# hangelwen/miR-PREFeR

Measured on AMD Instinct MI355X. Metric: precursor windows folded+filtered/sec (L=300), higher is better.
Workload: dtype int16/int32 (energies in 0.01 kcal/mol)

## Files before the change

mir-prefer_amd/csrc/fold_lds_common.h:

```cpp
#pragma once
#include <hip/hip_runtime.h>
#include <type_traits>
#include <tuple>
#include <cstdio>
#include "fold_epilogue.h"
#include "fold185_device.h"

namespace mirp {

#define LNT 1024
#define LNT2 512
#define LCAP 352
#define LDMAX 300
#define LSPAN 300
#define I16_INF 0x7fff
#define FIN_LIMIT 28000
#define FML_BIAS 31500
#define FML_MAX 1267
#define LSEG 384
#define KEY_BIAS 40000
#define KEY_NONE 0xffffffffu
#define KEY_INF (65535u << 10)
#define OTH_BIAS 2048

// ... 2 lines not shown
    short bulge[32];
    short internal_loop[32];
    short mismatchI[200], mismatchH[200], mismatchM[200], mismatch1nI[200], mismatch23I[200];
    unsigned char XB[176];
    unsigned char X1[176];
    short dangle5[40], dangle3[40];
    unsigned char rt2[28];
    short ML_closing, ML_intern, TerminalAU, ninio, MAX_NINIO, pad[3];
};
__host__ __device__ constexpr int xt_pslot(int s) { return s == 3 ? 3 : s == 4 ? 4 : 0; }
__host__ __device__ constexpr int xt_qslot(int s) { return s == 1 ? 1 : s == 3 ? 2 : s == 4 ? 1 : 0; }
__host__ __device__ constexpr int xt_pcode(int sp, int sp_m1) { return xt_pslot(sp) * 25 + sp_m1; }
__host__ __device__ constexpr int xt_qcode(int sq, int sq_p1) { return xt_qslot(sq) * 25 + sq_p1 * 5; }
static_assert(xt_pslot(1) + xt_qslot(4) == 1 && xt_pslot(2) + xt_qslot(3) == 2 && xt_pslot(3) + xt_qslot(2) == 3 && xt_pslot(3) + xt_qslot(4) == 4 &&
              xt_pslot(4) + xt_qslot(1) == 5 && xt_pslot(4) + xt_qslot(3) == 6, "inner-pair table slots");
template <class TAB>
__device__ inline void xt_fill(TAB& T, const FoldParams* __restrict__ P, int tid, int nt) {
    for (int x = tid; x < 175; x += nt) {
        const int slot = x / 25, a = (x % 25) / 5, b = x % 5;
        const int sp = slot == 1 ? 1 : slot == 2 ? 2 : (slot == 3 || slot == 4) ? 3 : 4, sq = slot == 1 ? 4 : slot == 2 ? 3 : slot == 3 ? 2 : slot == 4 ? 4 : slot == 5 ? 1 : 3;
        const int t2 = slot ? rtype_of(pair_type(sp, sq)) : 0;
        int xb = 0, x1 = 0;
        if (t2) {
            const int mi = P->mismatchI[t2][a][b];
            xb = (t2 > 2 ? P->TerminalAU : 0) - mi;
            x1 = P->mismatch1nI[t2][a][b] - mi;
        }
        T.XB[x] = (unsigned char)(xb + P->xb_bias); T.X1[x] = (unsigned char)(x1 + P->x1_bias);
    }
}
#define CSTR MIRP_RING_CSTR
#define MIRP_CK(d) ((d) % 3)
#define CRING_ROWS 33

struct LTab {
    static constexpr bool kTiled = true;
    const short* fml;
    const int* off;
    const short* carch;
    const unsigned short* tb;
    __device__ __forceinline__ int at(int d, int i) const { return off[(i - 1) >> 3] + ((i - 1) & 7) + 8 * (d - 4); }
    __device__ __forceinline__ int TB(int d, int i) const { return tb[at(d, i)]; }
    __device__ __forceinline__ int C(int d, int i) const { int v = carch[at(d, i)]; return v == I16_INF ? INF : v; }
    __device__ __forceinline__ int TBat(int o) const { return tb[o]; }
    __device__ __forceinline__ int Cat(int o) const { int v = carch[o]; return v == I16_INF ? INF : v; }
    __device__ __forceinline__ int Mat(int o) const { const int v = (unsigned short)fml[o]; return v == 65535 ? INF : v - FML_BIAS; }
    __device__ __forceinline__ int M(int d, int i) const {
        if (d < 4) return INF;
        const int v = (unsigned short)fml[at(d, i)];
        return v == 65535 ? INF : v - FML_BIAS;
    }
};

__device__ __forceinline__ int lds_mlstem(const LdsTables& T, const FoldParams* __restrict__ P, int type, int a, int b) {
    int e = T.ML_intern + (type > 2 ? T.TerminalAU : 0);
    if (a >= 0 && b >= 0) e += T.mismatchM[type * 25 + a * 5 + b];
    else if (a >= 0) e += P->dangle5[type][a];
    else if (b >= 0) e += P->dangle3[type][b];
    return e;
}

__device__ __forceinline__ int lds_intloop(const LdsTables& T, const FoldParams* __restrict__ P, int n1, int n2, int type, int type2,
                                           int si1, int sj1, int sp1, int sq1) {
    int nl = n1 > n2 ? n1 : n2, ns = n1 > n2 ? n2 : n1;
    if (nl == 0) return T.stack[type * 8 + type2];
    if (ns == 0) {
// ... 11 lines not shown
    }
    if (ns == 2) {
        if (nl == 2) return P->int22[type][type2][si1][sp1][sq1][sj1];
        if (nl == 3) return T.internal_loop[5] + T.ninio + T.mismatch23I[type * 25 + si1 * 5 + sj1] + T.mismatch23I[type2 * 25 + sq1 * 5 + sp1];
    }
    int x = (nl - ns) * T.ninio;
    return T.internal_loop[nl + ns] + (x < T.MAX_NINIO ? x : T.MAX_NINIO) + T.mismatchI[type * 25 + si1 * 5 + sj1] +
           T.mismatchI[type2 * 25 + sq1 * 5 + sp1];
}

__host__ __device__ constexpr int tri_off(int d, int n) { return 1 + (d - 4) * n - (d * (d - 1) / 2 - 6) + (((d - 4) + (n & 1)) >> 1); }
__host__ __device__ constexpr int tri_len(int d, int n) { return n - d > 0 ? (n - d) + ((n - d) & 1) : 0; }
__host__ __device__ constexpr int tri_len_any(int d, int n) { return (n - d) + ((n - d) & 1); }
__device__ inline void fill_tri_off(int* off, int n) {
    int o = 1;
    for (int d = 4; d <= LDMAX + 1; d++) { off[d] = o; o += tri_len(d, n); }
}

#define ARCH_RB ((LCAP + 7) / 8)
__host__ __device__ constexpr int arch_nd(int b, int n, int dcap) {
    int m = n - 1 - 8 * b;
    if (m > dcap) m = dcap;
    m -= 3;
    return m > 0 ? (m + 7) & ~7 : 0;
}
__host__ __device__ inline int arch_rowblk_off(int b, int n, int dcap) {
    int o = 0;
    for (int x = 0; x < b; x++) o += 8 * arch_nd(x, n, dcap);
    return o;
}

struct LdsLayout {
    unsigned fml, aux, S, seq, pax, qb2, list, tabs, misc, total, fml_bytes, code4, spec;
};
#define CODE_STR 384
static_assert(CODE_STR % 16 == 0 && (LCAP - 2) - 5 + MAXLOOP + 3 < CODE_STR, "pair-code reads of the first diagonals stay inside their copy");
__host__ __device__ constexpr unsigned lds_al(unsigned x) { return (x + 15u) & ~15u; }
#define FML_REGION_BYTES (lds_al((tri_off(LDMAX + 1, LCAP - 2) + 2) * 2))
#define POOL_MIN_CAP 1024
#define FRING_STR (LCAP + 2)
#ifndef MIRP_FILL_TWO_BYTES
#define MIRP_FILL_TWO_BYTES 71680
#endif
#ifndef MIRP_OVERLAP_EPI_WGS
#define MIRP_OVERLAP_EPI_WGS 1
#endif
#define MIRP_OVERLAP_EPI_LDS (16u * 1280u)
#define LDS_GRANULES(b) (((b) + 1279u) / 1280u)
#define LDS_TWO_BYTES ((unsigned)(MIRP_FILL_TWO_BYTES))
static_assert(2u * LDS_GRANULES(LDS_TWO_BYTES) + MIRP_OVERLAP_EPI_WGS * LDS_GRANULES(MIRP_OVERLAP_EPI_LDS) <= 128u, "two fill workgroups and the epilogue workgroups beside them share one CU's 160 KB");
template <int MODEL, bool SPARSE = false, bool TWO = false>
__host__ __device__ constexpr LdsLayout lds_layout() {
    static_assert(!TWO || (SPARSE && MODEL == 0), "two windows per CU: candidate-pool pass of the default model only");
    LdsLayout L{};
    unsigned o = 0;
    if (!SPARSE) { L.fml = o; L.fml_bytes = FML_REGION_BYTES; o += L.fml_bytes; }
    L.aux = o; o += lds_al(CRING_ROWS * CSTR * 2 + (MODEL ? 5 : 3) * LCAP * 2 + (SPARSE ? 6 : 5) * LCAP * 4);
    L.S = o; o += lds_al(LCAP + 8);
    L.seq = o; o += lds_al(LCAP + 8);
    if (SPARSE) {
        L.code4 = o; L.qb2 = o; L.pax = o + 4 * CODE_STR; o += 8 * CODE_STR;
    } else {
        L.pax = o; o += CODE_STR;
        L.qb2 = o; o += CODE_STR;
    }
    L.list = o; o += lds_al(3 * LSEG * 4);
    L.tabs = o; o += lds_al((unsigned)sizeof(LdsTables));
    L.misc = o; o += lds_al((48 + ARCH_RB + ((SPARSE && MODEL) ? 48 : 0)) * 4);
    if (TWO) { L.spec = o; o += lds_al(3 * CSTR * 2); }
    if (SPARSE) { L.fml = o; L.fml_bytes = (TWO ? LDS_TWO_BYTES : 160u * 1024u) - o; o += L.fml_bytes; }
    L.total = o;
    return L;
}
static_assert(lds_layout<0>().total <= 160 * 1024 && lds_layout<1>().total <= 160 * 1024, "fill kernel LDS budget");
static_assert(lds_layout<0, true, true>().total <= LDS_TWO_BYTES, "two workgroups of the candidate-pool pass must fit one CU's 160 KB");
static_assert((lds_layout<0, true, true>().fml_bytes - lds_al(2 * FRING_STR * 2)) / 6 >= 2 * POOL_MIN_CAP, "two-per-CU layout: room for the candidate pool behind the fML ring");

typedef const volatile __attribute__((address_space(3))) unsigned short* lds_vu16;
typedef const volatile __attribute__((address_space(3))) unsigned char* lds_vu8;
typedef const volatile __attribute__((address_space(3))) unsigned* lds_vu32;
#ifndef MIRP_A1_SMALLPACK
#define MIRP_A1_SMALLPACK 10
#endif
typedef unsigned short us2 __attribute__((ext_vector_type(2)));
typedef unsigned char pax_t;
typedef lds_vu8 lds_vpax;
struct A1 {
    const FoldParams* __restrict__ P;
    const LdsTables* T;
    const unsigned char* S;
    const unsigned short* cring;
    const pax_t* pax;
    const unsigned char* qbr;
    const unsigned char* code4 = nullptr;
    int r0, um, n;
    const int* __restrict__ rowtab;
    const unsigned short* rba = nullptr;
    unsigned w_lo = 0, w_hie = 0, w_hio = 0, w_sh = 0;
};

static_assert(CSTR % 2 == 0, "the aligned-dword ring reads need dword-aligned ring rows");
static_assert((CRING_ROWS - 1) * CSTR + (LCAP - 2) + 1 + MAXLOOP + 1 < CRING_ROWS * CSTR + 3 * LCAP, "the ring over-read stays inside the aux region");
#ifndef MIRP_RAMP_OLD_STRIDE
static_assert((LCAP - 2) - 6 + 1 + MAXLOOP + 1 < CSTR, "ramp-up diagonals: a lane's ring reads stay inside their row");
#endif

template <bool CHECK, int U>
__device__ __forceinline__ void a1_gen_row(const A1& a, const unsigned short* rb, unsigned& bg) {
    if constexpr (!CHECK && U >= 8) {
        lds_vu32 rq = (lds_vu32)(a.rba + a.rowtab[U]);
        constexpr int m1 = (U - 2) >> 1;
        unsigned dw[m1 + 2];
#pragma unroll
        for (int k = 1; k <= m1 + 1; k++) dw[k] = rq[k];
        const unsigned c1024 = 1024u;
#pragma unroll
        for (int m = 1; m <= m1; m++) {
            const unsigned re = __builtin_amdgcn_alignbit(dw[m + 1], dw[m], a.w_sh);
            unsigned e;
            asm("v_mad_u32_u16 %0, %1, %2, %3" : "=v"(e) : "v"(re), "v"(c1024), "s"(a.P->gen_key[U - 6][2 * m]));
            bg = e < bg ? e : bg;
            if (2 * m + 1 <= U - 2) {
                asm("v_mad_u32_u16 %0, %1, %2, %3 op_sel:[1,0,0,0]" : "=v"(e) : "v"(re), "v"(c1024), "s"(a.P->gen_key[U - 6][2 * m + 1]));
                bg = e < bg ? e : bg;
            }
        }
    } else
    if (!CHECK || U <= a.um) {
        lds_vu16 rp = (lds_vu16)(rb + a.rowtab[U]);
        unsigned v[U - 3];
#pragma unroll
        for (int n1 = 2; n1 <= U - 2; n1++) v[n1 - 2] = rp[n1];
#pragma unroll
        for (int n1 = 2; n1 <= U - 2; n1++) {
            const unsigned e = (v[n1 - 2] << 10) + a.P->gen_key[U - 6][n1];
// ... 210 lines not shown
    }
}

template <int N1, int N2>
__device__ __forceinline__ void a1_small(const A1& a, int i, int j, int type, int si1, int sj1, unsigned& best) {
    if (N1 + N2 <= a.um) {
        const int p = i + 1 + N1, q = j - 1 - N2;
        const unsigned g = a.cring[((a.r0 - N1 - N2) & 31) * CSTR + p];
        const int sp1 = a.S[p - 1], sq1 = a.S[q + 1];
        const int t2 = a.T->rt2[a.S[p] * 5 + a.S[q]];
        const int c = (int)g - 32768 - (int)a.T->mismatchI[t2 * 25 + sq1 * 5 + sp1];
        const int e = lds_intloop(*a.T, a.P, N1, N2, type, t2, si1, sj1, sp1, sq1) + c;
        const unsigned k = g == 65535u ? KEY_NONE : ((unsigned)(e + KEY_BIAS) << 10) | (unsigned)(N1 << 5 | N2);
        best = k < best ? k : best;
    }
}

template <int N1, int N2>
__device__ __forceinline__ void a1_small_g(const A1& a, int i, int j, int type, int si1, int sj1, int& raw, int& cc) {
    raw = 0; cc = INF;
    if (N1 + N2 <= a.um) {
        const int p = i + 1 + N1, q = j - 1 - N2;
        const unsigned g = a.cring[((a.r0 - N1 - N2) & 31) * CSTR + p];
        const int sp1 = a.S[p - 1], sq1 = a.S[q + 1];
        const int t2 = a.T->rt2[a.S[p] * 5 + a.S[q]];
        cc = g == 65535u ? INF : (int)g - 32768 - (int)a.T->mismatchI[t2 * 25 + sq1 * 5 + sp1];
        if (N1 == 1 && N2 == 1) raw = a.P->int11[type][t2][si1][sj1];
        else if (N1 == 1 && N2 == 2) raw = a.P->int21[type][t2][si1][sq1][sj1];
        else if (N1 == 2 && N2 == 1) raw = a.P->int21[t2][type][sq1][si1][sp1];
        else raw = a.P->int22[type][t2][si1][sp1][sq1][sj1];
    }
}

#define A1_CHUNK 10
template <int K>
__device__ __forceinline__ unsigned a1_add_byte(unsigned base, unsigned w) {
    unsigned r;
    if constexpr (K == 0) asm("v_add_u32_sdwa %0, %1, %2 dst_sel:DWORD dst_unused:UNUSED_PAD src0_sel:DWORD src1_sel:BYTE_0" : "=v"(r) : "v"(base), "v"(w));
    else if constexpr (K == 1) asm("v_add_u32_sdwa %0, %1, %2 dst_sel:DWORD dst_unused:UNUSED_PAD src0_sel:DWORD src1_sel:BYTE_1" : "=v"(r) : "v"(base), "v"(w));
    else if constexpr (K == 2) asm("v_add_u32_sdwa %0, %1, %2 dst_sel:DWORD dst_unused:UNUSED_PAD src0_sel:DWORD src1_sel:BYTE_2" : "=v"(r) : "v"(base), "v"(w));
    else asm("v_add_u32_sdwa %0, %1, %2 dst_sel:DWORD dst_unused:UNUSED_PAD src0_sel:DWORD src1_sel:BYTE_3" : "=v"(r) : "v"(base), "v"(w));
    return r;
}
template <int N, int K = 0>
__device__ __forceinline__ void a1_gather4(unsigned tab_idx, const unsigned (&dw)[(N + 3) / 4], int (&x)[N]) {
    if constexpr (K < N) {
        x[K] = *(lds_vu8)(size_t)a1_add_byte<K & 3>(tab_idx, dw[K >> 2]);
        a1_gather4<N, K + 1>(tab_idx, dw, x);
    }
}
template <int N>
__device__ __forceinline__ void a1_codes4(const A1& a, int which, int A, const unsigned char* tab, unsigned idx, int (&x)[N]) {
    typedef const volatile __attribute__((address_space(3))) unsigned* lds_vu32;
    const int c = A & 3;
    lds_vu32 p = (lds_vu32)(a.code4 + which * 4 * CODE_STR + c * (CODE_STR - 1) + A);
    unsigned dw[(N + 3) / 4];
#pragma unroll
    for (int t = 0; t < (N + 3) / 4; t++) dw[t] = p[t];
    const unsigned tab_idx = (unsigned)(size_t)(__attribute__((address_space(3))) const unsigned char*)tab + idx;
    a1_gather4<N>(tab_idx, dw, x);
}
template <int LO, int HI>
__device__ __forceinline__ void a1_b0f(const A1& a, int i, int j, unsigned& best) {
    if constexpr (HI - LO + 1 > A1_CHUNK) { a1_b0f<LO, LO + A1_CHUNK - 1>(a, i, j, best); a1_b0f<LO + A1_CHUNK, HI>(a, i, j, best); }
    else {
        constexpr int N = HI - LO + 1;
        const unsigned idxp = a.pax[i + 1];
        lds_vu8 ql = (lds_vu8)(a.qbr + (a.n + 2 - j));
        const unsigned short* rb = a.cring + i + 1;
        const unsigned char* xb = a.T->XB;
        unsigned code[N], g[N];
        int x[N];
#pragma unroll
        for (int k = 0; k < N; k++) g[k] = rb[a.rowtab[LO + k]];
#pragma unroll
        for (int k = 0; k < N; k++) if (!a.code4) code[k] = ql[LO + k];
        if (a.code4) a1_codes4<N>(a, 0, a.n + 2 - j + LO, xb, idxp, x);
        else {
#pragma unroll
            for (int k = 0; k < N; k++) x[k] = xb[idxp + code[k]];
        }
#pragma unroll
        for (int k = 0; k < N; k++) { const unsigned e = ((g[k] + (unsigned)x[k]) << 10) + a.P->kb0_key[LO + k]; best = e < best ? e : best; }
    }
}
template <int LO, int HI>
__device__ __forceinline__ void a1_b1f(const A1& a, int i, int j, unsigned& best) {
    if constexpr (HI - LO + 1 > A1_CHUNK) { a1_b1f<LO, LO + A1_CHUNK - 1>(a, i, j, best); a1_b1f<LO + A1_CHUNK, HI>(a, i, j, best); }
    else {
        constexpr int N = HI - LO + 1;
        const unsigned idxq = a.qbr[a.n + 2 - j];
        lds_vpax pl = (lds_vpax)(a.pax + i + 1);
        const unsigned short* rb = a.cring + i + 1;
        const unsigned char* xb = a.T->XB;
        unsigned code[N], g[N];
        int x[N];
#pragma unroll
        for (int k = 0; k < N; k++) g[k] = rb[a.rowtab[LO + k] + (LO + k)];
#pragma unroll
        for (int k = 0; k < N; k++) if (!a.code4) code[k] = pl[LO + k];
        if (a.code4) a1_codes4<N>(a, 1, i + 1 + LO, xb, idxq, x);
        else {
#pragma unroll
            for (int k = 0; k < N; k++) x[k] = xb[idxq + code[k]];
        }
#pragma unroll
        for (int k = 0; k < N; k++) { const unsigned e = ((g[k] + (unsigned)x[k]) << 10) + a.P->kb1_key[LO + k]; best = e < best ? e : best; }
    }
}
template <int LO, int HI>
__device__ __forceinline__ void a1_i0f(const A1& a, int i, int j, unsigned& best) {
    if constexpr (HI - LO + 1 > A1_CHUNK) { a1_i0f<LO, LO + A1_CHUNK - 1>(a, i, j, best); a1_i0f<LO + A1_CHUNK, HI>(a, i, j, best); }
    else {
        constexpr int N = HI - LO + 1;
        const unsigned idxp = a.pax[i + 2];
        lds_vu8 ql = (lds_vu8)(a.qbr + (a.n + 2 - j));
        const unsigned short* rb = a.cring + i + 2;
        const unsigned char* xb = a.T->X1;
        unsigned code[N], g[N];
        int x[N];
#pragma unroll
        for (int k = 0; k < N; k++) g[k] = rb[a.rowtab[LO + k + 1]];
#pragma unroll
        for (int k = 0; k < N; k++) if (!a.code4) code[k] = ql[LO + k];
        if (a.code4) a1_codes4<N>(a, 0, a.n + 2 - j + LO, xb, idxp, x);
        else {
#pragma unroll
            for (int k = 0; k < N; k++) x[k] = xb[idxp + code[k]];
        }
#pragma unroll
        for (int k = 0; k < N; k++) { const unsigned e = ((g[k] + (unsigned)x[k]) << 10) + a.P->k1n0_key[LO + k]; best = e < best ? e : best; }
    }
}
template <int LO, int HI>
__device__ __forceinline__ void a1_i1f(const A1& a, int i, int j, unsigned& best) {
    if constexpr (HI - LO + 1 > A1_CHUNK) { a1_i1f<LO, LO + A1_CHUNK - 1>(a, i, j, best); a1_i1f<LO + A1_CHUNK, HI>(a, i, j, best); }
    else {
        constexpr int N = HI - LO + 1;
        const unsigned idxq = a.qbr[a.n + 3 - j];
        lds_vpax pl = (lds_vpax)(a.pax + i + 1);
        const unsigned short* rb = a.cring + i + 1;
        const unsigned char* xb = a.T->X1;
        unsigned code[N], g[N];
        int x[N];
#pragma unroll
        for (int k = 0; k < N; k++) g[k] = rb[a.rowtab[LO + k + 1] + (LO + k)];
#pragma unroll
        for (int k = 0; k < N; k++) if (!a.code4) code[k] = pl[LO + k];
        if (a.code4) a1_codes4<N>(a, 1, i + 1 + LO, xb, idxq, x);
        else {
#pragma unroll
            for (int k = 0; k < N; k++) x[k] = xb[idxq + code[k]];
        }
#pragma unroll
        for (int k = 0; k < N; k++) { const unsigned e = ((g[k] + (unsigned)x[k]) << 10) + a.P->k1n1_key[LO + k]; best = e < best ? e : best; }
    }
}

__device__ __forceinline__ unsigned a1_small_key(unsigned g, int mm_inner, int e_loop, unsigned code) {
    const int e = e_loop + (int)g - 32768 - mm_inner;
    return g == 65535u ? KEY_NONE : ((unsigned)(e + KEY_BIAS) << 10) | code;
}
__device__ __forceinline__ unsigned a1_small14f(const A1& a, int i, int j, int type, bool ahead) {
    lds_vu8 Sv = (lds_vu8)a.S;
    const int s_i = Sv[i], s_i1 = Sv[i + 1], s_i2 = Sv[i + 2], s_j3 = Sv[j - 3], s_j2 = Sv[j - 2], s_j1 = Sv[j - 1], s_j = Sv[j];
    const unsigned short* rb = a.cring;
    const unsigned g00 = rb[((a.r0) & 31) * CSTR + i + 1], g01 = rb[((a.r0 - 1) & 31) * CSTR + i + 1], g10 = rb[((a.r0 - 1) & 31) * CSTR + i + 2];
    const unsigned g11 = rb[((a.r0 - 2) & 31) * CSTR + i + 2], g12 = rb[((a.r0 - 3) & 31) * CSTR + i + 2];
    const int t00 = rtype_of(pair_type(s_i1, s_j1)), t01 = rtype_of(pair_type(s_i1, s_j2)), t10 = rtype_of(pair_type(s_i2, s_j1));
    const int t11 = rtype_of(pair_type(s_i2, s_j2)), t12 = rtype_of(pair_type(s_i2, s_j3));
    const LdsTables& T = *a.T;
    const int m00 = T.mismatchI[t00 * 25 + s_j * 5 + s_i], m01 = T.mismatchI[t01 * 25 + s_j1 * 5 + s_i], m10 = T.mismatchI[t10 * 25 + s_j * 5 + s_i1];
    const int m11 = T.mismatchI[t11 * 25 + s_j1 * 5 + s_i1], m12 = T.mismatchI[t12 * 25 + s_j2 * 5 + s_i1];
    const int st00 = T.stack[type * 8 + t00], st01 = T.stack[type * 8 + t01], st10 = T.stack[type * 8 + t10], b1 = T.bulge[1];
    const int r11 = a.P->int11[type][t11][s_i1][s_j1];
    const int r12 = a.P->int21[type][t12][s_i1][s_j2][s_j1];
    unsigned res = a1_small_key(g01, m01, b1 + st01, 0u << 5 | 1u);
    unsigned k = a1_small_key(g10, m10, b1 + st10, 1u << 5 | 0u); res = k < res ? k : res;
    k = a1_small_key(g00, m00, st00, 0u); if (!ahead) res = k < res ? k : res;
    k = a1_small_key(g11, m11, r11, 1u << 5 | 1u); res = k < res ? k : res;
    k = a1_small_key(g12, m12, r12, 1u << 5 | 2u); res = k < res ? k : res;
    return res;
// ... 24 lines not shown
```

mir-prefer_amd/csrc/fold_lds_kernel_body.h:

```cpp
    extern __shared__ __align__(16) unsigned char smem[];
    constexpr bool TWO = NT != LNT;
    static_assert(NT == LNT || NT == LNT2, "workgroup size");
    constexpr int NW = NT / 64;
    constexpr LdsLayout LY = lds_layout<MODEL, SPARSE, TWO>();
#ifdef MIRP_DIAG
    const bool light = light_clocks_arg != 0;
    long long* const dbg_cycles = dbg_cycles_arg;
#else
    constexpr bool light = false;
    constexpr long long* dbg_cycles = nullptr;
    (void)light_clocks_arg; (void)dbg_cycles_arg;
#endif
    constexpr int DMLR = MODEL ? 5 : 3;
#define ENT_OUTER(mmo, mm1) ((unsigned)(((mmo) & 1023) | (((mm1) & 1023) << 10)))
    const int tau_s = __builtin_amdgcn_readfirstlane(P->TerminalAU);
    constexpr int GEN_WD = 5;
    long long tA = 0, tB = 0, tS = 0, tE = 0, t0 = 0;
    long long tR = 0, nR = 0, nB = 0;
    long long wB = 0, wA1 = 0, wA2 = 0, wW = 0, wt = 0;
    unsigned short* fml = (unsigned short*)(smem + LY.fml);
    unsigned short* cring = (unsigned short*)(smem + LY.aux);
    short* dmlring = (short*)(cring + CRING_ROWS * CSTR);
    int* acc = (int*)(dmlring + DMLR * LCAP);
    constexpr int NACC = SPARSE ? 6 : 5;
    auto mdec_of = [&](int d) -> int* { return acc + (3 + (SPARSE ? d % 3 : (d & 1))) * LCAP; };
    unsigned char* S = smem + LY.S;
    unsigned char* seq = smem + LY.seq;
    pax_t* pax = (pax_t*)(smem + LY.pax);
    unsigned char* qbr = smem + LY.qb2;
    unsigned char* code4 = SPARSE ? smem + LY.code4 : nullptr;
#ifdef MIRP_RAMP_CHECKED
    constexpr bool RAMPF = false;
#else
    constexpr bool RAMPF = TWO;
#endif
    short* spec = RAMPF ? (short*)(smem + LY.spec) : (short*)(cring + 29 * CSTR);
    using list_t = unsigned;
    list_t* list = (list_t*)(smem + LY.list);
    LdsTables& T = *(LdsTables*)(smem + LY.tabs);
    int* misc = (int*)(smem + LY.misc);
    int* lcnt = misc + 16;
    int* rbt = misc + 48;
    const int tid = threadIdx.x, lane = tid & 63;
    const int wave = __builtin_amdgcn_readfirstlane(tid >> 6);
    if (wave < (TWO ? 6 : 12)) __builtin_amdgcn_s_setprio(1);
    const int nc = CSTR;
    auto list_append = [&](int dd, int i, int t, int oi) {
        const unsigned long long bal = __ballot(t != 0);
        if (bal) {
            int base = 0;
            if (lane == 0) base = atomicAdd(&lcnt[dd % 6], (int)__popcll(bal));
            base = __builtin_amdgcn_readfirstlane(base);
            if (t) list[(dd % 3) * LSEG + base + __popcll(bal & ((1ull << lane) - 1ull))] = (list_t)((unsigned)i | ((unsigned)t << 9) | ((unsigned)oi << 12));
        }
    };

    for (int x = tid; x < 64; x += NT) T.stack[x] = (short)min(P->stack[x >> 3][x & 7], (int)I16_INF);
    for (int x = tid; x < 31; x += NT) { T.bulge[x] = (short)min(P->bulge[x], (int)I16_INF); T.internal_loop[x] = (short)min(P->internal_loop[x], (int)I16_INF); }
    for (int x = tid; x < 200; x += NT) {
        int t = x / 25, a = (x % 25) / 5, b = x % 5;
        T.mismatchI[x] = (short)min(P->mismatchI[t][a][b], (int)I16_INF); T.mismatchH[x] = (short)min(P->mismatchH[t][a][b], (int)I16_INF);
        T.mismatchM[x] = (short)P->mismatchM[t][a][b]; T.mismatch1nI[x] = (short)min(P->mismatch1nI[t][a][b], (int)I16_INF);
        T.mismatch23I[x] = (short)min(P->mismatch23I[t][a][b], (int)I16_INF);
// ... 28 lines not shown
        unsigned short* tb_out = reinterpret_cast<unsigned short*>(carch + 2 * slab_shorts);
        if (dbg_cycles && tid == 0) t0 = clock64();
        int xki = 0;
        if constexpr (MODEL != 0) {
            if (n >= 1 && n <= LCAP - 2)
                for (int x = tid; x < n; x += NT) { const unsigned u = seqs[o0 + x] & 0xdfu; if (u == 'X' || u == 'K' || u == 'I') misc[4] = 1; }
            __syncthreads();
            xki = misc[4];
            __syncthreads();
            if (tid == 0) misc[4] = 0;
        }
        if (n < 1 || n > LCAP - 2 || xki) {
            if (tid == 0) {
                out_nlines[win] = 0; out_mfe[win] = 0; out_status[win] = 0; win_state[win] = 0;
                if (n >= 1) { unsigned int k = atomicAdd(fallback_count, 1u); fallback_list[k] = win_base + win; }
            }
        } else if (SPARSE && pool_cap < POOL_MIN_CAP) {
            if (tid == 0) { out_nlines[win] = 0; out_mfe[win] = 0; out_status[win] = 0; win_state[win] = 0; dense_list[atomicAdd(dense_count, 1u)] = win; }
        } else {
        const int D = (span - 1 < n - 1) ? span - 1 : n - 1;
        const int Dm = MODEL ? ((span < n - 1) ? span : n - 1) : D;
        for (int x = tid; x <= n + 1; x += NT) {
            unsigned char ch = 0;
            if (x >= 1 && x <= n) {
                ch = seqs[o0 + x - 1];
                if (ch >= 'a' && ch <= 'z') ch -= 32;
                if (ch == 'T') ch = 'U';
            }
            seq[x] = ch;
            S[x] = ch == 'A' ? 1 : ch == 'C' ? 2 : ch == 'G' ? 3 : ch == 'U' ? 4 : 0;
        }
        for (int x = tid; x < DMLR * LCAP; x += NT) dmlring[x] = (short)I16_INF;
        if constexpr (RAMPF) {
            static_assert((CRING_ROWS * CSTR) % 2 == 0, "ring initialisation by dwords");
            unsigned* cr32 = reinterpret_cast<unsigned*>(cring);
            for (int x = tid; x < CRING_ROWS * CSTR / 2; x += NT) cr32[x] = 0xffffffffu;
        }
        for (int x = tid; x < NACC * LCAP; x += NT) acc[x] = x >= 3 * LCAP ? INF : (int)KEY_NONE;
        if (tid == 0) {
            misc[1] = 0; misc[2] = 0; misc[3] = 0;
            if constexpr (SPARSE && MODEL != 0) for (int x = 0; x < 44; x++) pbits[x] = 0;
            for (int x = 0; x < 6; x++) lcnt[x] = 0;
        }
        if (tid >= 64 && tid < 64 + ARCH_RB) rbt[tid - 64] = arch_rowblk_off(tid - 64, n, span);
        __syncthreads();
        if (tid == 0) { S[0] = S[n]; S[n + 1] = S[1]; }
        for (int x = tid; x <= n; x += NT) {
            short s3 = -32768, s4 = -32768, s6 = -32768;
            if (x >= 1) {
                if (x + 4 <= n)
                    for (int k = 0; k < P->n_tri; k++) { bool m = true; for (int t = 0; t < 5; t++) m = m && (seq[x + t] == (unsigned char)P->tri[k][t]); if (m && s3 == -32768) s3 = (short)P->triE[k]; }
                if (x + 5 <= n)
                    for (int k = 0; k < P->n_tetra; k++) { bool m = true; for (int t = 0; t < 6; t++) m = m && (seq[x + t] == (unsigned char)P->tetra[k][t]); if (m && s4 == -32768) s4 = (short)P->tetraE[k]; }
                if (x + 7 <= n)
                    for (int k = 0; k < P->n_hexa; k++) { bool m = true; for (int t = 0; t < 8; t++) m = m && (seq[x + t] == (unsigned char)P->hexa[k][t]); if (m && s6 == -32768) s6 = (short)P->hexaE[k]; }
            }
            if (MODEL) s4 = s4 == -32768 ? (short)0 : s4;
            spec[x] = s3; spec[nc + x] = s4; spec[2 * nc + x] = s6;
            if (x >= 1) {
                pax[x] = (pax_t)xt_pcode(S[x], x > 1 ? (int)S[x - 1] : 0);
                qbr[n + 1 - x] = (unsigned char)xt_qcode(S[x], x < n ? (int)S[x + 1] : 0);
            }
        }
        for (int dd = 4; dd <= 6 && dd <= D; dd++) {
            int t = 0, oi = 0;
            if (tid < n - dd) {
                t = pair_type(S[tid + 1], S[tid + 1 + dd]);
                const int x = t * 25 + S[tid + 2] * 5 + S[tid + dd];
                oi = ENT_OUTER((int)T.mismatchI[x], (int)T.mismatch1nI[x]);
// ... 195 lines not shown
            const bool swap_order = !SPARSE && (wave & 1);
            auto splits = [&]() { if constexpr (SPARSE && MODEL != 0) splits_sparse185(); else if constexpr (TWO) splits_sparse2(); else if constexpr (SPARSE) splits_sparse(); else splits_dense(); };
            if (swap_order) splits();
            if constexpr (TWO) a2_prefetch();
            if (dbg_cycles && lane == 0 && !light) wt = clock64();
            if (d >= 6 && d <= D) {
                const list_t* clist = list + (d % 3) * LSEG;
                const bool mix = d - 2 - (TURN + 1) >= MAXLOOP && d + 1 <= D;
                const int ncp = a1_ncp;
                const int done = a1_done;
                const int rem = ncp - done;
                const int nblk = (rem + 63) >> 6;
                int ncp2;
                if (lc_have) { asm volatile("s_waitcnt lgkmcnt(0)" : "+v"(lc_pre) : : "memory"); ncp2 = __builtin_amdgcn_readfirstlane(lc_pre); }
                else ncp2 = __builtin_amdgcn_readfirstlane(lcnt[(d + 1) % 6]);
                a1_ncp = ncp2;
                const int room = nblk * 64 - rem;
                const int take2 = mix ? (room < ncp2 ? room : ncp2) : 0;
                a1_done = take2;
                unsigned* ckey2 = reinterpret_cast<unsigned*>(acc + MIRP_CK(d + 1) * LCAP);
                unsigned aent = 0;
                {
                    const int ka = lane - (64 - room);
                    if (ka >= 0 && ka < take2) aent = list[((d + 1) % 3) * LSEG + ka];
                }
#define MIRP_XROWS15 9, 7
#define MIRP_XROWS8 8
#define MIRP_XROWS9 10
                A1 a;
                a.P = P; a.T = &T; a.S = S; a.cring = cring; a.pax = pax; a.qbr = qbr; a.code4 = code4; a.n = n;
#define MIRP_A1_BLOCK()                                                                                                        \
                    {                                                                                                          \
                        int r0 = d - 2, um = d - 2 - (TURN + 1) < MAXLOOP ? d - 2 - (TURN + 1) : MAXLOOP;                      \
                        asm volatile("" : "+s"(r0), "+s"(um));                                                                 \
                        a.r0 = r0; a.um = um;                                                                                  \
                        a.rowtab = P->ring_rowoff[r0 & 31];                                                                    \
                    }                                                                                                          \
                    const int k = blk * 64 + lane;                                                                             \
                    const bool own = k < rem, ahead = !own && aent != 0;          \
                    const bool act = own || ahead;                                                                             \
                    unsigned ent = own ? clist[done + k] : ahead ? aent : (1u | (1u << 9));
#ifdef MIRP_A1_FUSED
                const int role1st = wave < 4 ? wave : wave < 6 ? wave + 10 : wave + 6, role2nd = wave < 4 ? wave + 8 : wave;
                for (int blk = 0; blk < nblk; blk++) {
                    MIRP_A1_BLOCK()
                    unsigned best = KEY_NONE;
                    int npass = 2;
                    asm volatile("" : "+s"(npass));
                    for (int pass = 0; pass < npass; pass++) {
                    const int role = pass ? role2nd : role1st;
                    asm volatile("" : "+v"(ent));
#define MIRP_A1_ROLE14_HERE (wave == 4)
#else
#pragma nounroll
                for (int pass = 0; pass < (TWO ? 2 : 1); pass++) {
                const int role = TWO ? (wave < 4 ? wave + 8 * pass : wave < 6 ? (pass ? wave : wave + 10) : (pass ? wave : wave + 6))
                                     : wave < 4 ? wave : wave < 6 ? wave + 10 : wave < 12 ? wave + 2 : wave - 8;
                for (int blk = 0; blk < nblk; blk++) {
                    MIRP_A1_BLOCK()
#define MIRP_A1_ROLE14_HERE (role == 14)
#endif
                    const int i = ent & 511, type = (ent >> 9) & 7, j = i + d + (ahead ? 1 : 0);
                    a.cring = cring + (ahead ? CSTR : 0);
                    unsigned* ck = ahead ? ckey2 : ckey;
                    unsigned res = KEY_NONE;
                    int au1 = 0, mmo = 0, mm1 = 0;
                    if (role < 14 || MODEL == 0) {
                        au1 = type > 2 ? tau_s : 0;
                        mmo = ((int)(ent << 10)) >> 22; mm1 = ((int)ent) >> 22;
                    }
                    if (role < 8) {
#define MIRP_GEN(CK)                                                                      \
    switch (role) {                                                                       \
    case 0: res = MIRP_A1G<CK MIRP_A1WD, 30, 23>(a, i, j, mmo); if (CK) a1_i1<CK, 28, 29>(a, i, j, xi); else a1_i1f<28, 29>(a, i, j, xi); break;      \
    case 1: res = MIRP_A1G<CK MIRP_A1WD, 29, 24>(a, i, j, mmo); if (CK) a1_i1<CK, 25, 27>(a, i, j, xi); else a1_i1f<25, 27>(a, i, j, xi); break;      \
    case 2: res = MIRP_A1G<CK MIRP_A1WD, 28, 25>(a, i, j, mmo); if (CK) a1_i0<CK, 26, 29>(a, i, j, xi); else a1_i0f<26, 29>(a, i, j, xi); break;      \
    case 3: res = MIRP_A1G<CK MIRP_A1WD, 27, 26>(a, i, j, mmo); if (CK) a1_b1<CK, 26, 30>(a, i, j, xb); else a1_b1f<26, 30>(a, i, j, xb); break;      \
    case 4: res = MIRP_A1G<CK MIRP_A1WD, MIRP_ROWS4>(a, i, j, mmo); break;                    \
    case 5: res = MIRP_A1G<CK MIRP_A1WD, MIRP_ROWS5>(a, i, j, mmo); break;                    \
    case 6: res = MIRP_A1G<CK MIRP_A1WD, MIRP_ROWS6>(a, i, j, mmo); break;                    \
    default: res = MIRP_A1G<CK MIRP_A1WD, MIRP_ROWS7>(a, i, j, mmo); break;               \
    }
#define MIRP_XGEN(CK)                                                                     \
    switch (role) {                                                                       \
    case 15: rx = MIRP_A1G<CK MIRP_A1WD, MIRP_XROWS15>(a, i, j, mmo); break;                         \
    case 8: rx = MIRP_A1G<CK MIRP_A1WD, MIRP_XROWS8>(a, i, j, mmo); break;                           \
    case 9: rx = MIRP_A1G<CK MIRP_A1WD, MIRP_XROWS9>(a, i, j, mmo); break;                           \
    default: break;                                                                       \
    }
                        unsigned xb = KEY_INF, xi = KEY_INF;
                        if constexpr (MODEL == 0) {
#define MIRP_A1G a1_generic_w
#define MIRP_A1WD , GEN_WD
#define MIRP_ROWS4 22, 17, 12
#define MIRP_ROWS5 21, 18, 11
#define MIRP_ROWS6 20, 16, 13
#define MIRP_ROWS7 19, 15, 14, 6
                            if (RAMPF || a.um >= MAXLOOP) { MIRP_GEN(false) } else { MIRP_GEN(true) }
#undef MIRP_A1G
#undef MIRP_A1WD
#undef MIRP_ROWS4
#undef MIRP_ROWS5
#undef MIRP_ROWS6
#undef MIRP_ROWS7
                        } else {
#define MIRP_A1G a1_generic
#define MIRP_A1WD
#define MIRP_ROWS4 22, 17, 12, 7
#define MIRP_ROWS5 21, 18, 11, 8
#define MIRP_ROWS6 20, 16, 13, 9
#define MIRP_ROWS7 19, 15, 14, 10, 6
                            if (RAMPF || a.um >= MAXLOOP) { MIRP_GEN(false) } else { MIRP_GEN(true) }
#undef MIRP_A1G
#undef MIRP_A1WD
#undef MIRP_ROWS4
#undef MIRP_ROWS5
#undef MIRP_ROWS6
#undef MIRP_ROWS7
                        }
                        if (role < 4) {
                            const unsigned rb = a1_key(xb, -32768 - OTH_BIAS + au1);
                            const unsigned ri = a1_key(xi, -32768 - OTH_BIAS + mm1);
                            res = rb < res ? rb : res;
                            res = ri < res ? ri : res;
                        }
#undef MIRP_GEN
                    } else if (role < 14) {
                        unsigned bb = KEY_INF, bi = KEY_INF;
                        if (RAMPF || a.um >= MAXLOOP) {
                            switch (role) {
                            case 8: a1_b0f<2, 18>(a, i, j, bb); break;
                            case 9: a1_b0f<19, 30>(a, i, j, bb); a1_b1f<2, 6>(a, i, j, bb); break;
                            case 10: a1_b1f<7, 22>(a, i, j, bb); break;
                            case 11: a1_b1f<23, 25>(a, i, j, bb); a1_i0f<3, 15>(a, i, j, bi); break;
                            case 12: a1_i0f<16, 25>(a, i, j, bi); a1_i1f<3, 8>(a, i, j, bi); break;
                            default: a1_i1f<9, 24>(a, i, j, bi); break;
                            }
                        } else {
                            switch (role) {
                            case 8: a1_b0<true, 2, 18>(a, i, j, bb); break;
                            case 9: a1_b0<true, 19, 30>(a, i, j, bb); a1_b1<true, 2, 6>(a, i, j, bb); break;
                            case 10: a1_b1<true, 7, 22>(a, i, j, bb); break;
                            case 11: a1_b1<true, 23, 25>(a, i, j, bb); a1_i0<true, 3, 15>(a, i, j, bi); break;
                            case 12: a1_i0<true, 16, 25>(a, i, j, bi); a1_i1<true, 3, 8>(a, i, j, bi); break;
                            default: a1_i1<true, 9, 24>(a, i, j, bi); break;
                            }
                        }
                        const unsigned rb = a1_key(bb, -32768 - OTH_BIAS + au1);
                        const unsigned ri = a1_key(bi, -32768 - OTH_BIAS + mm1);
                        res = rb < ri ? rb : ri;
                    } else if (RAMPF || a.um >= MAXLOOP) {
                        res = role == 14 ? a1_small14f(a, i, j, type, ahead) : a1_small15f(a, i, j, type);
                    } else {
                        const int si1 = S[i + 1], sj1 = S[j - 1];
                        int ra, ca, rb2, cb2;
                        unsigned ka, kb2;
                        if (role == 14) {
                            a1_small_g<1, 1>(a, i, j, type, si1, sj1, ra, ca); a1_small_g<1, 2>(a, i, j, type, si1, sj1, rb2, cb2);
                            unsigned r00 = KEY_NONE;
                            a1_small<0, 0>(a, i, j, type, si1, sj1, r00); a1_small<0, 1>(a, i, j, type, si1, sj1, res); a1_small<1, 0>(a, i, j, type, si1, sj1, res);
                            if (!ahead) res = r00 < res ? r00 : res;
                            ka = 1 << 5 | 1; kb2 = 1 << 5 | 2;
                        } else {
                            a1_small_g<2, 1>(a, i, j, type, si1, sj1, ra, ca); a1_small_g<2, 2>(a, i, j, type, si1, sj1, rb2, cb2);
                            a1_small<2, 3>(a, i, j, type, si1, sj1, res); a1_small<3, 2>(a, i, j, type, si1, sj1, res);
                            ka = 2 << 5 | 1; kb2 = 2 << 5 | 2;
                        }
                        if (ca < INF) { const unsigned k = ((unsigned)(ra + ca + KEY_BIAS) << 10) | ka; res = k < res ? k : res; }
                        if (cb2 < INF) { const unsigned k = ((unsigned)(rb2 + cb2 + KEY_BIAS) << 10) | kb2; res = k < res ? k : res; }
// ... 99 lines not shown
                    cv = h < cint ? h : cint;
                    if (dmlv != I16_INF) {
                        const int e = dmlv + mlc + mli + (rt > 2 ? tau : 0) + mmMc;
                        cv = e < cv ? e : cv;
                    }
                    if (cint < INF && cint == cv && h != cv) tb = (int)(kk & 1023u) + 1;
                }
                int m = INF;
                {
                    const int a = fa == 65535 ? INF : fa - FML_BIAS, b = fb == 65535 ? INF : fb - FML_BIAS;
                    m = a < b ? a : b;
                }
                if (type) {
                    const int stem = mli + au + ((i > 1 && j < n) ? mmMs : (i > 1) ? dg5 : (j < n) ? dg3 : 0);
                    const int e = cv + stem;
                    if constexpr (SPARSE) cand = cv < INF && e < m && e < md;
                    m = e < m ? e : m;
                }
                m = md < m ? md : m;
                if constexpr (SPARSE) {
                    cbal = __ballot(cand != 0);
                    if (cbal && lane == 0) {
                        const unsigned pa = (unsigned)(size_t)(__attribute__((address_space(3))) int*)&misc[3];
                        asm volatile("ds_add_rtn_u32 %0, %1, %2" : "=v"(cbase) : "v"(pa), "v"((int)__popcll(cbal)) : "memory");
                    }
                    cent = (unsigned)(i - 1) | ((unsigned)j << 9);
                }
                if ((cv < INF && (cv > FIN_LIMIT || cv < -FIN_LIMIT)) || (m < INF && (m > FML_MAX || m < -FML_BIAS)) ||
                    (md < INF && (md > FIN_LIMIT || md < -FIN_LIMIT))) misc[1] = 1;
                const short c16 = cv >= INF ? (short)I16_INF : (short)cv;
                const unsigned short m16 = m >= INF ? (unsigned short)65535 : (unsigned short)(m + FML_BIAS);
                const unsigned short g16 = cv < INF ? (unsigned short)(cv + mmI + 32768) : (unsigned short)65535;
                cring[(d & 31) * CSTR + i] = g16;
                if ((d & 31) == 0) cring[32 * CSTR + i] = g16;
                carch[abase + 8 * d] = c16;
                tb_out[abase + 8 * d] = (unsigned short)tb;
                fml[od + i] = m16;
                if constexpr (TWO) fml_out[abase + 8 * d] = (short)m16;
                dmlring[(d % DMLR) * LCAP + i] = md >= INF ? (short)I16_INF : (short)md;
                ckey[i] = KEY_NONE;
                if constexpr (SPARSE) { mdec_of(d + 2)[i] = INF; cval = m16; }
                else mdec[i] = INF;
            }
            if constexpr (SPARSE) {
                if (cbal) {
                    asm volatile("s_waitcnt lgkmcnt(0)" : "+v"(cbase) : : "memory");
                    const int at = __builtin_amdgcn_readfirstlane(cbase) + (int)__popcll(cbal & ((1ull << lane) - 1ull));
                    if (cand) {
                        if (at < pool_cap) { poolA[at] = cent; poolB[at] = (unsigned short)cval; }
                        else misc[2] = 1;
                    }
                }
            }
            asm volatile("s_waitcnt lgkmcnt(0)" : "+v"(lbase) : : "memory");
            const int lb = __builtin_amdgcn_readfirstlane(lbase);
            if (lt) list[(d % 3) * LSEG + lb + __popcll(lbal & ((1ull << lane) - 1ull))] = (list_t)((unsigned)(x + 1) | ((unsigned)lt << 9) | ((unsigned)ent_terms << 12));
        };
        auto phaseB1 = [&](const int d) {
            const int ncell = n - d;
            unsigned* ckey = reinterpret_cast<unsigned*>(acc + MIRP_CK(d) * LCAP);
            int* mdec = mdec_of(d);
            int cand = 0; unsigned cent = 0, cval = 0;
            if constexpr (SPARSE) { if (tid < 11) pbits[((d + 1) & 3) * 11 + tid] = 0; }
            const int hp_u = P->hairpinE[d - 1 < MIRP_HP_MAX ? d - 1 : MIRP_HP_MAX - 1];
            const int od = tri_off(d, n), od1 = tri_off(d - 1, n);
            const int x = tid;
            int lt = 0, lbase = 0, loi = 0, ent_terms = 0;
// ... 230 lines not shown
```

Measured before the change: 397,500.

## Mirror ring rows so two-per-CU bulge reads use immediate offsets

Extends the circular C-ring for the two-windows-per-CU layout with ten mirrored rows past row 32, so that a chunk of up to ten consecutive ring rows is contiguous. The bulge and interior-loop chunk reads can then use one base row plus compile-time immediate offsets instead of loading per-row offsets from a row table. The table base address for the code gather also skips an address-space cast. The cost is extra LDS for the mirrored rows and extra stores on each diagonal that falls in the mirrored range.

```diff
diff --git a/mir-prefer_amd/csrc/fold_lds_common.h b/mir-prefer_amd/csrc/fold_lds_common.h
--- a/mir-prefer_amd/csrc/fold_lds_common.h
+++ b/mir-prefer_amd/csrc/fold_lds_common.h
@@ -58,6 +58,9 @@
 #define CSTR MIRP_RING_CSTR
 #define MIRP_CK(d) ((d) % 3)
 #define CRING_ROWS 33
+#define A1_CHUNK 10
+#define CRING_ROWS_WIN (32 + A1_CHUNK)
+template <bool TWO> __host__ __device__ constexpr int cring_rows() { return TWO ? CRING_ROWS_WIN : CRING_ROWS; }
 
 struct LTab {
     static constexpr bool kTiled = true;
@@ -135,6 +138,7 @@
 
 struct LdsLayout {
     unsigned fml, aux, S, seq, pax, qb2, list, tabs, misc, total, fml_bytes, code4, spec;
+    int ring_rows;
 };
 #define CODE_STR 384
 static_assert(CODE_STR % 16 == 0 && (LCAP - 2) - 5 + MAXLOOP + 3 < CODE_STR, "pair-code reads of the first diagonals stay inside their copy");
@@ -158,7 +162,8 @@
     LdsLayout L{};
     unsigned o = 0;
     if (!SPARSE) { L.fml = o; L.fml_bytes = FML_REGION_BYTES; o += L.fml_bytes; }
-    L.aux = o; o += lds_al(CRING_ROWS * CSTR * 2 + (MODEL ? 5 : 3) * LCAP * 2 + (SPARSE ? 6 : 5) * LCAP * 4);
+    L.ring_rows = cring_rows<TWO>();
+    L.aux = o; o += lds_al(L.ring_rows * CSTR * 2 + (MODEL ? 5 : 3) * LCAP * 2 + (SPARSE ? 6 : 5) * LCAP * 4);
     L.S = o; o += lds_al(LCAP + 8);
     L.seq = o; o += lds_al(LCAP + 8);
     if (SPARSE) {
@@ -203,7 +208,9 @@
 };
 
 static_assert(CSTR % 2 == 0, "the aligned-dword ring reads need dword-aligned ring rows");
-static_assert((CRING_ROWS - 1) * CSTR + (LCAP - 2) + 1 + MAXLOOP + 1 < CRING_ROWS * CSTR + 3 * LCAP, "the ring over-read stays inside the aux region");
+template <bool TWO> __host__ __device__ constexpr bool cring_overread_ok() { return (cring_rows<TWO>() - 1) * CSTR + (LCAP - 2) + 1 + MAXLOOP + 1 < cring_rows<TWO>() * CSTR + 3 * LCAP; }
+static_assert(cring_overread_ok<false>() && cring_overread_ok<true>(), "the ring over-read stays inside the aux region");
+static_assert(lds_layout<0, true, true>().ring_rows == CRING_ROWS_WIN && lds_layout<0>().ring_rows == CRING_ROWS && lds_layout<1, true>().ring_rows == CRING_ROWS, "only the two-per-CU layout mirrors a chunk of rows");
 #ifndef MIRP_RAMP_OLD_STRIDE
 static_assert((LCAP - 2) - 6 + 1 + MAXLOOP + 1 < CSTR, "ramp-up diagonals: a lane's ring reads stay inside their row");
 #endif
@@ -480,7 +487,6 @@
     }
 }
 
-#define A1_CHUNK 10
 template <int K>
 __device__ __forceinline__ unsigned a1_add_byte(unsigned base, unsigned w) {
     unsigned r;
@@ -497,7 +503,10 @@
         a1_gather4<N, K + 1>(tab_idx, dw, x);
     }
 }
-template <int N>
+#ifndef MIRP_A1_TABLO
+#define MIRP_A1_TABLO 1
+#endif
+template <int N, bool WIN = false>
 __device__ __forceinline__ void a1_codes4(const A1& a, int which, int A, const unsigned char* tab, unsigned idx, int (&x)[N]) {
     typedef const volatile __attribute__((address_space(3))) unsigned* lds_vu32;
     const int c = A & 3;
@@ -505,12 +514,20 @@
     unsigned dw[(N + 3) / 4];
 #pragma unroll
     for (int t = 0; t < (N + 3) / 4; t++) dw[t] = p[t];
-    const unsigned tab_idx = (unsigned)(size_t)(__attribute__((address_space(3))) const unsigned char*)tab + idx;
+    unsigned tab_idx;
+    if constexpr (WIN && MIRP_A1_TABLO) tab_idx = (unsigned)(size_t)tab + idx;
+    else tab_idx = (unsigned)(size_t)(__attribute__((address_space(3))) const unsigned char*)tab + idx;
     a1_gather4<N>(tab_idx, dw, x);
 }
-template <int LO, int HI>
+template <int UMAX>
+__device__ __forceinline__ int a1_win_row(const A1& a) {
+    int r0 = a.r0;
+    asm volatile("" : "+s"(r0));
+    return ((r0 - UMAX) & 31) * CSTR;
+}
+template <bool WIN, int LO, int HI>
 __device__ __forceinline__ void a1_b0f(const A1& a, int i, int j, unsigned& best) {
-    if constexpr (HI - LO + 1 > A1_CHUNK) { a1_b0f<LO, LO + A1_CHUNK - 1>(a, i, j, best); a1_b0f<LO + A1_CHUNK, HI>(a, i, j, best); }
+    if constexpr (HI - LO + 1 > A1_CHUNK) { a1_b0f<WIN, LO, LO + A1_CHUNK - 1>(a, i, j, best); a1_b0f<WIN, LO + A1_CHUNK, HI>(a, i, j, best); }
     else {
         constexpr int N = HI - LO + 1;
         const unsigned idxp = a.pax[i + 1];
@@ -519,11 +536,17 @@
         const unsigned char* xb = a.T->XB;
         unsigned code[N], g[N];
         int x[N];
-#pragma unroll
-        for (int k = 0; k < N; k++) g[k] = rb[a.rowtab[LO + k]];
+        if constexpr (WIN) {
+            const unsigned short* rw = rb + a1_win_row<HI>(a);
+#pragma unroll
+            for (int k = 0; k < N; k++) g[k] = rw[(N - 1 - k) * CSTR];
+        } else {
+#pragma unroll
+            for (int k = 0; k < N; k++) g[k] = rb[a.rowtab[LO + k]];
+        }
 #pragma unroll
         for (int k = 0; k < N; k++) if (!a.code4) code[k] = ql[LO + k];
-        if (a.code4) a1_codes4<N>(a, 0, a.n + 2 - j + LO, xb, idxp, x);
+        if (a.code4) a1_codes4<N, WIN>(a, 0, a.n + 2 - j + LO, xb, idxp, x);
         else {
 #pragma unroll
             for (int k = 0; k < N; k++) x[k] = xb[idxp + code[k]];
@@ -532,9 +555,9 @@
         for (int k = 0; k < N; k++) { const unsigned e = ((g[k] + (unsigned)x[k]) << 10) + a.P->kb0_key[LO + k]; best = e < best ? e : best; }
     }
 }
-template <int LO, int HI>
+template <bool WIN, int LO, int HI>
 __device__ __forceinline__ void a1_b1f(const A1& a, int i, int j, unsigned& best) {
-    if constexpr (HI - LO + 1 > A1_CHUNK) { a1_b1f<LO, LO + A1_CHUNK - 1>(a, i, j, best); a1_b1f<LO + A1_CHUNK, HI>(a, i, j, best); }
+    if constexpr (HI - LO + 1 > A1_CHUNK) { a1_b1f<WIN, LO, LO + A1_CHUNK - 1>(a, i, j, best); a1_b1f<WIN, LO + A1_CHUNK, HI>(a, i, j, best); }
     else {
         constexpr int N = HI - LO + 1;
         const unsigned idxq = a.qbr[a.n + 2 - j];
@@ -543,11 +566,17 @@
         const unsigned char* xb = a.T->XB;
         unsigned code[N], g[N];
         int x[N];
-#pragma unroll
-        for (int k = 0; k < N; k++) g[k] = rb[a.rowtab[LO + k] + (LO + k)];
+        if constexpr (WIN) {
+            const unsigned short* rw = rb + a1_win_row<HI>(a);
+#pragma unroll
+            for (int k = 0; k < N; k++) g[k] = rw[(N - 1 - k) * CSTR + (LO + k)];
+        } else {
+#pragma unroll
+            for (int k = 0; k < N; k++) g[k] = rb[a.rowtab[LO + k] + (LO + k)];
+        }
 #pragma unroll
         for (int k = 0; k < N; k++) if (!a.code4) code[k] = pl[LO + k];
-        if (a.code4) a1_codes4<N>(a, 1, i + 1 + LO, xb, idxq, x);
+        if (a.code4) a1_codes4<N, WIN>(a, 1, i + 1 + LO, xb, idxq, x);
         else {
 #pragma unroll
             for (int k = 0; k < N; k++) x[k] = xb[idxq + code[k]];
@@ -556,9 +585,9 @@
         for (int k = 0; k < N; k++) { const unsigned e = ((g[k] + (unsigned)x[k]) << 10) + a.P->kb1_key[LO + k]; best = e < best ? e : best; }
     }
 }
-template <int LO, int HI>
+template <bool WIN, int LO, int HI>
 __device__ __forceinline__ void a1_i0f(const A1& a, int i, int j, unsigned& best) {
-    if constexpr (HI - LO + 1 > A1_CHUNK) { a1_i0f<LO, LO + A1_CHUNK - 1>(a, i, j, best); a1_i0f<LO + A1_CHUNK, HI>(a, i, j, best); }
+    if constexpr (HI - LO + 1 > A1_CHUNK) { a1_i0f<WIN, LO, LO + A1_CHUNK - 1>(a, i, j, best); a1_i0f<WIN, LO + A1_CHUNK, HI>(a, i, j, best); }
     else {
         constexpr int N = HI - LO + 1;
         const unsigned idxp = a.pax[i + 2];
@@ -567,11 +596,17 @@
         const unsigned char* xb = a.T->X1;
         unsigned code[N], g[N];
         int x[N];
-#pragma unroll
-        for (int k = 0; k < N; k++) g[k] = rb[a.rowtab[LO + k + 1]];
+        if constexpr (WIN) {
+            const unsigned short* rw = rb + a1_win_row<HI + 1>(a);
+#pragma unroll
+            for (int k = 0; k < N; k++) g[k] = rw[(N - 1 - k) * CSTR];
+        } else {
+#pragma unroll
+            for (int k = 0; k < N; k++) g[k] = rb[a.rowtab[LO + k + 1]];
+        }
 #pragma unroll
         for (int k = 0; k < N; k++) if (!a.code4) code[k] = ql[LO + k];
-        if (a.code4) a1_codes4<N>(a, 0, a.n + 2 - j + LO, xb, idxp, x);
+        if (a.code4) a1_codes4<N, WIN>(a, 0, a.n + 2 - j + LO, xb, idxp, x);
         else {
 #pragma unroll
             for (int k = 0; k < N; k++) x[k] = xb[idxp + code[k]];
@@ -580,9 +615,9 @@
         for (int k = 0; k < N; k++) { const unsigned e = ((g[k] + (unsigned)x[k]) << 10) + a.P->k1n0_key[LO + k]; best = e < best ? e : best; }
     }
 }
-template <int LO, int HI>
+template <bool WIN, int LO, int HI>
 __device__ __forceinline__ void a1_i1f(const A1& a, int i, int j, unsigned& best) {
-    if constexpr (HI - LO + 1 > A1_CHUNK) { a1_i1f<LO, LO + A1_CHUNK - 1>(a, i, j, best); a1_i1f<LO + A1_CHUNK, HI>(a, i, j, best); }
+    if constexpr (HI - LO + 1 > A1_CHUNK) { a1_i1f<WIN, LO, LO + A1_CHUNK - 1>(a, i, j, best); a1_i1f<WIN, LO + A1_CHUNK, HI>(a, i, j, best); }
     else {
         constexpr int N = HI - LO + 1;
         const unsigned idxq = a.qbr[a.n + 3 - j];
@@ -591,11 +626,17 @@
         const unsigned char* xb = a.T->X1;
         unsigned code[N], g[N];
         int x[N];
-#pragma unroll
-        for (int k = 0; k < N; k++) g[k] = rb[a.rowtab[LO + k + 1] + (LO + k)];
+        if constexpr (WIN) {
+            const unsigned short* rw = rb + a1_win_row<HI + 1>(a);
+#pragma unroll
+            for (int k = 0; k < N; k++) g[k] = rw[(N - 1 - k) * CSTR + (LO + k)];
+        } else {
+#pragma unroll
+            for (int k = 0; k < N; k++) g[k] = rb[a.rowtab[LO + k + 1] + (LO + k)];
+        }
 #pragma unroll
         for (int k = 0; k < N; k++) if (!a.code4) code[k] = pl[LO + k];
-        if (a.code4) a1_codes4<N>(a, 1, i + 1 + LO, xb, idxq, x);
+        if (a.code4) a1_codes4<N, WIN>(a, 1, i + 1 + LO, xb, idxq, x);
         else {
 #pragma unroll
             for (int k = 0; k < N; k++) x[k] = xb[idxq + code[k]];
diff --git a/mir-prefer_amd/csrc/fold_lds_kernel_body.h b/mir-prefer_amd/csrc/fold_lds_kernel_body.h
--- a/mir-prefer_amd/csrc/fold_lds_kernel_body.h
+++ b/mir-prefer_amd/csrc/fold_lds_kernel_body.h
@@ -20,7 +20,7 @@
     long long wB = 0, wA1 = 0, wA2 = 0, wW = 0, wt = 0;
     unsigned short* fml = (unsigned short*)(smem + LY.fml);
     unsigned short* cring = (unsigned short*)(smem + LY.aux);
-    short* dmlring = (short*)(cring + CRING_ROWS * CSTR);
+    short* dmlring = (short*)(cring + LY.ring_rows * CSTR);
     int* acc = (int*)(dmlring + DMLR * LCAP);
     constexpr int NACC = SPARSE ? 6 : 5;
     auto mdec_of = [&](int d) -> int* { return acc + (3 + (SPARSE ? d % 3 : (d & 1))) * LCAP; };
@@ -29,6 +29,11 @@
     pax_t* pax = (pax_t*)(smem + LY.pax);
     unsigned char* qbr = smem + LY.qb2;
     unsigned char* code4 = SPARSE ? smem + LY.code4 : nullptr;
+#ifndef MIRP_A1_WIN
+#define MIRP_A1_WIN 1
+#endif
+    constexpr bool A1WIN = TWO && MIRP_A1_WIN != 0;
+    static_assert(!A1WIN || LY.ring_rows == CRING_ROWS_WIN, "immediate-offset ring reads need the mirror rows");
 #ifdef MIRP_RAMP_CHECKED
     constexpr bool RAMPF = false;
 #else
@@ -123,9 +128,9 @@
         }
         for (int x = tid; x < DMLR * LCAP; x += NT) dmlring[x] = (short)I16_INF;
         if constexpr (RAMPF) {
-            static_assert((CRING_ROWS * CSTR) % 2 == 0, "ring initialisation by dwords");
+            static_assert((LY.ring_rows * CSTR) % 2 == 0, "ring initialisation by dwords");
             unsigned* cr32 = reinterpret_cast<unsigned*>(cring);
-            for (int x = tid; x < CRING_ROWS * CSTR / 2; x += NT) cr32[x] = 0xffffffffu;
+            for (int x = tid; x < LY.ring_rows * CSTR / 2; x += NT) cr32[x] = 0xffffffffu;
         }
         for (int x = tid; x < NACC * LCAP; x += NT) acc[x] = x >= 3 * LCAP ? INF : (int)KEY_NONE;
         if (tid == 0) {
@@ -387,7 +392,7 @@
 #define MIRP_A1_BLOCK()                                                                                                        \
                     {                                                                                                          \
                         int r0 = d - 2, um = d - 2 - (TURN + 1) < MAXLOOP ? d - 2 - (TURN + 1) : MAXLOOP;                      \
-                        asm volatile("" : "+s"(r0), "+s"(um));                                                                 \
+                        if (!A1WIN) asm volatile("" : "+s"(r0), "+s"(um));                                                     \
                         a.r0 = r0; a.um = um;                                                                                  \
                         a.rowtab = P->ring_rowoff[r0 & 31];                                                                    \
                     }                                                                                                          \
@@ -427,10 +432,10 @@
                     if (role < 8) {
 #define MIRP_GEN(CK)                                                                      \
     switch (role) {                                                                       \
-    case 0: res = MIRP_A1G<CK MIRP_A1WD, 30, 23>(a, i, j, mmo); if (CK) a1_i1<CK, 28, 29>(a, i, j, xi); else a1_i1f<28, 29>(a, i, j, xi); break;      \
-    case 1: res = MIRP_A1G<CK MIRP_A1WD, 29, 24>(a, i, j, mmo); if (CK) a1_i1<CK, 25, 27>(a, i, j, xi); else a1_i1f<25, 27>(a, i, j, xi); break;      \
-    case 2: res = MIRP_A1G<CK MIRP_A1WD, 28, 25>(a, i, j, mmo); if (CK) a1_i0<CK, 26, 29>(a, i, j, xi); else a1_i0f<26, 29>(a, i, j, xi); break;      \
-    case 3: res = MIRP_A1G<CK MIRP_A1WD, 27, 26>(a, i, j, mmo); if (CK) a1_b1<CK, 26, 30>(a, i, j, xb); else a1_b1f<26, 30>(a, i, j, xb); break;      \
+    case 0: res = MIRP_A1G<CK MIRP_A1WD, 30, 23>(a, i, j, mmo); if (CK) a1_i1<CK, 28, 29>(a, i, j, xi); else a1_i1f<A1WIN, 28, 29>(a, i, j, xi); break;      \
+    case 1: res = MIRP_A1G<CK MIRP_A1WD, 29, 24>(a, i, j, mmo); if (CK) a1_i1<CK, 25, 27>(a, i, j, xi); else a1_i1f<A1WIN, 25, 27>(a, i, j, xi); break;      \
+    case 2: res = MIRP_A1G<CK MIRP_A1WD, 28, 25>(a, i, j, mmo); if (CK) a1_i0<CK, 26, 29>(a, i, j, xi); else a1_i0f<A1WIN, 26, 29>(a, i, j, xi); break;      \
+    case 3: res = MIRP_A1G<CK MIRP_A1WD, 27, 26>(a, i, j, mmo); if (CK) a1_b1<CK, 26, 30>(a, i, j, xb); else a1_b1f<A1WIN, 26, 30>(a, i, j, xb); break;      \
     case 4: res = MIRP_A1G<CK MIRP_A1WD, MIRP_ROWS4>(a, i, j, mmo); break;                    \
     case 5: res = MIRP_A1G<CK MIRP_A1WD, MIRP_ROWS5>(a, i, j, mmo); break;                    \
     case 6: res = MIRP_A1G<CK MIRP_A1WD, MIRP_ROWS6>(a, i, j, mmo); break;                    \
@@ -484,12 +489,12 @@
                         unsigned bb = KEY_INF, bi = KEY_INF;
                         if (RAMPF || a.um >= MAXLOOP) {
                             switch (role) {
-                            case 8: a1_b0f<2, 18>(a, i, j, bb); break;
-                            case 9: a1_b0f<19, 30>(a, i, j, bb); a1_b1f<2, 6>(a, i, j, bb); break;
-                            case 10: a1_b1f<7, 22>(a, i, j, bb); break;
-                            case 11: a1_b1f<23, 25>(a, i, j, bb); a1_i0f<3, 15>(a, i, j, bi); break;
-                            case 12: a1_i0f<16, 25>(a, i, j, bi); a1_i1f<3, 8>(a, i, j, bi); break;
-                            default: a1_i1f<9, 24>(a, i, j, bi); break;
+                            case 8: a1_b0f<A1WIN, 2, 18>(a, i, j, bb); break;
+                            case 9: a1_b0f<A1WIN, 19, 30>(a, i, j, bb); a1_b1f<A1WIN, 2, 6>(a, i, j, bb); break;
+                            case 10: a1_b1f<A1WIN, 7, 22>(a, i, j, bb); break;
+                            case 11: a1_b1f<A1WIN, 23, 25>(a, i, j, bb); a1_i0f<A1WIN, 3, 15>(a, i, j, bi); break;
+                            case 12: a1_i0f<A1WIN, 16, 25>(a, i, j, bi); a1_i1f<A1WIN, 3, 8>(a, i, j, bi); break;
+                            default: a1_i1f<A1WIN, 9, 24>(a, i, j, bi); break;
                             }
                         } else {
                             switch (role) {
@@ -655,7 +660,11 @@
                 const unsigned short m16 = m >= INF ? (unsigned short)65535 : (unsigned short)(m + FML_BIAS);
                 const unsigned short g16 = cv < INF ? (unsigned short)(cv + mmI + 32768) : (unsigned short)65535;
                 cring[(d & 31) * CSTR + i] = g16;
+#ifdef MIRP_NO_RING_MIRROR
                 if ((d & 31) == 0) cring[32 * CSTR + i] = g16;
+#else
+                if ((d & 31) < LY.ring_rows - 32) cring[(32 + (d & 31)) * CSTR + i] = g16;
+#endif
                 carch[abase + 8 * d] = c16;
                 tb_out[abase + 8 * d] = (unsigned short)tb;
                 fml[od + i] = m16;
```

New measurement: 402,600 (median of 6 runs). 1.3% higher.
